# arnab39/equiadapt

Hardware: AMD Instinct MI355X
Metric: canonicalize+invert images/sec (224x224 C8) (higher is better)
Workload: dtype f32 (resampling / FFT / accumulation in fp32; the network's channel contraction as 2xfp16 split of every fp32 operand (within one fp32 ulp), 3 exact products, fp32 accumulate -- closer to fp64 than the fp32 matrix instruction, see step_ms_by_gemm_form); 1 GPU; configs[1]: 224x224x3 synthetic, C8, GroupEquivariantImageCanonicalization + ESCNNEquivariantNetwork in e2cnn's LAYER SHAPES (32 fields x 8 = 256 ch, k5, 3 layers, crop 0.8, resize 96) with this repository's own filter-bank parameterisation (bilinear-rotated banks; e2cnn's steerable basis is not restated -- e2cnn-trained weights enter via load_exported_dense), forward, then invert_canonicalization; batch_per_gpu=256, global_batch=256, parallelism=dp1 (no collective in the forward path)

## Files before the change

equiadapt_amd/csrc/lift_fft.hip:

```cpp
#include <cstdlib>

#include "eqa_common.hpp"

#ifndef EQA_LF_AUX
#define EQA_LF_AUX 2
#endif

namespace {

#include "fft_common.inc"

typedef float f32x4 __attribute__((ext_vector_type(4)));
typedef unsigned u32x4 __attribute__((ext_vector_type(4)));

struct alignas(4) LfPixel { float c[3]; };
__device__ __forceinline__ void lf_fetch_pixel(float (&p)[3], const float* __restrict__ x, unsigned off, bool ok) {
  const LfPixel v = *reinterpret_cast<const LfPixel*>(reinterpret_cast<const char*>(x) + (ok ? off : 0u));
#pragma unroll
  for (int c = 0; c < 3; ++c) p[c] = v.c[c];
}
__device__ __forceinline__ float lf_pixel_or_zero(float v, bool ok) { return ok ? v : 0.0f; }

#ifdef EQA_LF_CLOCK
__device__ unsigned long long g_lf_clock[64];
__device__ __forceinline__ int lf_clock_slot(int wave) { return wave == 8 ? 0 : wave == 1 ? 1 : wave == 0 ? 2 : wave == 6 ? 3 : wave == 11 ? 4 : -1; }
#define LF_CLOCK_BEGIN() const bool lfc_on = blockIdx.x == 0 && (threadIdx.x & 63) == 0 && lf_clock_slot(wave) >= 0; \
  if (blockIdx.x == 0 && (threadIdx.x & 63) == 0) { unsigned hw_; asm volatile("s_getreg_b32 %0, hwreg(HW_REG_HW_ID)" : "=s"(hw_)); g_lf_clock[40 + wave] = hw_; } \
  unsigned long long lfc_t = __builtin_readcyclecounter(); unsigned long long lfc_s[16] = {0, 0, 0, 0, 0, 0, 0, 0, 0, 0, 0, 0, 0, 0, 0, 0}
#define LF_CLOCK(i) do { const unsigned long long n_ = __builtin_readcyclecounter(); lfc_s[i] += n_ - lfc_t; lfc_t = n_; } while (0)
#define LF_CLOCK_END() do { if (lfc_on) for (int i_ = 0; i_ < 8; ++i_) g_lf_clock[8 * lf_clock_slot(wave) + i_] = lfc_s[i_]; } while (0)
#else
#define LF_CLOCK_BEGIN() do { } while (0)
#define LF_CLOCK(i) do { } while (0)
#define LF_CLOCK_END() do { } while (0)
#endif

constexpr int kLfThreads = 768;
constexpr int kLfCh = 16;
constexpr int kLfSteps = 19;
constexpr int kLfQuadPitch = 196;
constexpr int kLfRowPitch = 784;
constexpr int kLfTileFloats = kFftN * kLfRowPitch;
constexpr int kLfSubRows = 16;
constexpr int kLfPatchRows = kLfSubRows + 4, kLfPatchPitch = 156;
constexpr int kLfPatchFloats = kLfPatchRows * kLfPatchPitch;
constexpr int kLfLdsFloats = kLfTileFloats + kLfPatchFloats;
constexpr int kLfStagers = 6 * 64;
constexpr int kLfPre = (kLfPatchFloats + kLfStagers - 1) / kLfStagers;

__device__ __forceinline__ void lf_slot(int n, int& ky, int& e, bool& spare) {
  spare = n == 75;
  const bool lo = n < 70;
  const int r = n % 14;
  ky = lo ? n / 14 : min(n - 70, 4);
  e = lo ? (r >> 1) + 8 * (r & 1) : 7;
}

struct LfItem {
  unsigned grp, m;
  int gy0, gx0;
  size_t img;
};

__device__ __forceinline__ LfItem lf_item(unsigned work, int ngrp, int TY, int TX) {
  LfItem it;
  it.grp = work % ngrp;
#ifdef EQA_LF_XCDGRP
  if (ngrp == 16) it.grp = 2 * (it.grp % 8) + it.grp / 8;
#endif
  it.m = work / ngrp;
  const unsigned tx = it.m % TX, ty = (it.m / TX) % TY;
  it.img = it.m / ((unsigned)TX * TY);
  it.gy0 = kFftO * (int)ty;
  it.gx0 = kFftO * (int)tx;
  return it;
}

enum { kConv = 0, kCols = 1, kRowp = 2 };

#ifndef EQA_LF_H2_DEAL
#define EQA_LF_H2_DEAL 1
#endif
constexpr int kLhDeal = EQA_LF_H2_DEAL;
constexpr int kLhRun0 = kLhDeal == 0 ? 3 : 6, kLhRun1 = kLhDeal == 0 ? 6 : 0;
constexpr int kLhFirstConv = kLhDeal == 0 ? 8 : 6;
constexpr bool kLhConvRowsInTail = kLhDeal != 0;
struct LfRun { int y0, t0, y1, t1; bool cross; };
__host__ __device__ constexpr LfRun lf_h2_run(int wave, int ) {
  if (kLhDeal == 0) {
    const bool cross = wave == 9 || wave == 10;
    const int y0 = (wave == 8 || wave == 10) ? 0 : (wave == 9 ? 9 : 3), t0 = (wave == 8 || wave == 9) ? 0 : 2;
    return LfRun{y0, t0, cross ? (wave == 9 ? 0 : 6) : y0 + 3, cross ? 1 : t0, cross};
  }
  const bool lone = wave == 8 || wave == 9;
  const int y0 = ((lone ? wave == 9 : wave >= 10) ? 6 : 0), t0 = lone ? 0 : 1 + (wave & 1);
  return LfRun{y0, t0, y0 + kLhRun0, t0, false};
}
constexpr bool lf_h2_deal_covers() {
  int n[3][12] = {};
  for (int sub = 0; sub < 4; ++sub) {
    for (int w = kLhFirstConv; w < 12; ++w) {
      const LfRun r = lf_h2_run(w, sub);
      if (r.cross != (kLhRun1 > 0 && r.t1 != r.t0)) return false;
      for (int k = 0; k < kLhRun0 + kLhRun1; ++k) {
        const int y = k < kLhRun0 ? r.y0 + k : r.y1 + k - kLhRun0, t = k < kLhRun0 ? r.t0 : r.t1;
        if (y < 0 || y >= 12 || t < 0 || t >= 3) return false;
        ++n[t][y];
      }
    }
  }
  for (int t = 0; t < 3; ++t)
    for (int y = 0; y < 12; ++y)
      if (n[t][y] != 4) return false;
  return true;
}
static_assert(lf_h2_deal_covers(), "FORM 2: a tile of the sub-phase is left to no wave or taken by two");

#if EQA_LF_H2_DEAL != 0
__device__ __forceinline__ int lf_h2_rows(int wave, int s) { return s < 4 ? 0 : 4 * wave; }
#elif defined(EQA_LF_H2_ROWS_IN_SUB)
__device__ __forceinline__ int lf_h2_rows(int wave, int s) {
  if (s < 4) return wave == 6 ? (1 | ((s & 1) ? 4 : 0)) : (wave == 7 ? (2 | ((s & 1) ? 0 : 4)) : 0);
  return wave == 6 ? 36 : wave == 7 ? 40 : wave == 4 ? 44 : -1;
}
#else
__device__ __forceinline__ int lf_h2_rows(int wave, int s) {
  if (s < 4) return wave == 6 ? 1 : (wave == 7 ? 2 : 0);
  return wave == 6 ? 36 : wave == 7 ? 40 : wave == 0 ? 8 : wave == 4 ? 20 : wave == 1 ? 32 : wave == 5 ? 44 : -1;
}
#endif

template <class F, int... Is>
__device__ __forceinline__ void lf_for_const(F&& f, std::integer_sequence<int, Is...>) {
  (f(std::integral_constant<int, Is>()), ...);
}

constexpr int kLpRowB = 53 * 8;
constexpr int kLpPlaneB = 8 * kLpRowB;
constexpr int kLpPatchB = 3 * kLpPlaneB;
constexpr int kLpLdsBytes = kLfTileFloats * 4 + kLpPatchB;
constexpr int kLhRowB = 52 * 8;
constexpr int kLhRing = 16;
constexpr int kLhPlaneB = kLhRing * kLhRowB;
constexpr int kLhPatchB = 2 * kLhPlaneB;
constexpr int kLhLdsBytes = kLfTileFloats * 4 + kLhPatchB;
constexpr int kLhSubRows = 12;
constexpr int kLhPre = 3;
typedef _Float16 lf_f16x8 __attribute__((ext_vector_type(8)));
typedef _Float16 lf_f16x4 __attribute__((ext_vector_type(4)));
typedef __bf16 lf_bf16x8 __attribute__((ext_vector_type(8)));
typedef __bf16 lf_bf16x4 __attribute__((ext_vector_type(4)));
__device__ __forceinline__ void lf_split3(float x, __bf16& p1, __bf16& p2, __bf16& p3) {
  p1 = (__bf16)x;
  const float r1 = x - (float)p1;
  p2 = (__bf16)r1;
  p3 = (__bf16)(r1 - (float)p2);
}

template <int ROLE, int FORM>
__device__ __forceinline__ void lift5_fft48_body(const float* __restrict__ x, const float* __restrict__ bank, const float* __restrict__ bias,
                                                 int relu, float* __restrict__ V, int H0, int W0, int C, int TY, int TX, size_t Mp,
                                                 unsigned nwork, unsigned v_bytes, unsigned x_bytes, unsigned bank_bytes,
                                                 float* __restrict__ dcmax, const float* __restrict__ xbound, int nxbound, float w_scale) {
  constexpr bool COLS = ROLE == kCols;
  constexpr bool PIECES = FORM == 3;
  constexpr bool H2 = FORM == 2;
  constexpr int NSUB = PIECES ? 12 : (H2 ? 4 : 3);
  constexpr int SUBROWS = kFftN / NSUB;
  constexpr int NGRP = 12 / NSUB;
  extern __shared__ float lds[];
  float* const tile = lds;
  float* const patch = lds + kLfTileFloats;
  const int tid = threadIdx.x;
  const int lane = tid & 63;
  const int wave = __builtin_amdgcn_readfirstlane(tid >> 6);
  const int j = lane & 15, q = lane >> 4;
  const int ngrp = C / kLfCh;
  const int H1 = H0 - 4, W1 = W0 - 4;
  const unsigned nblk = gridDim.x;
  const unsigned patch_b = (unsigned)(kLfTileFloats * 4);
  LF_CLOCK_BEGIN();

  const __amdgpu_buffer_rsrc_t xr = __builtin_amdgcn_make_buffer_rsrc(const_cast<float*>(x), 0, x_bytes, 0x00020000);
  float pre[COLS ? kLfPre : 1];
  auto prefetch = [&](const LfItem& it, int sub, bool live) {
    if constexpr (COLS) {
      int tq = tid;
      asm volatile("" : "+v"(tq));
#pragma unroll
      for (int i = 0; i < kLfPre; ++i) {
        const int idx = tq + kLfStagers * i;
        const int pr = idx / kLfPatchPitch, pc = idx - pr * kLfPatchPitch;
        const int gy = it.gy0 + kLfSubRows * sub + pr, gxc = it.gx0 * 3 + pc;
        const bool ok = live && idx < kLfPatchFloats && gy < H0 && gxc < W0 * 3;
        const unsigned off = ok ? (unsigned)(((it.img * H0 + gy) * (size_t)(W0 * 3) + gxc) * 4) : 0xfffffff0u;
        pre[i] = __builtin_bit_cast(float, __builtin_amdgcn_raw_buffer_load_b32(xr, off, 0, 0));
      }
    }
  };
  auto stage = [&]() {
    if constexpr (COLS) {
#pragma unroll
      for (int i = 0; i < kLfPre; ++i) {
        const int idx = tid + kLfStagers * i;
        if (idx < kLfPatchFloats) patch[idx] = pre[i];
      }
    }
  };

  float preg[COLS && PIECES ? 2 : 1][3];
  bool preg_ok[2] = {false, false};
  auto prefetch_grp = [&](const LfItem& it, int g, int which, bool live) {
    if constexpr (COLS && PIECES) {
      int tq = tid;
      asm volatile("" : "+v"(tq));
      const int pr = tq / 52, px = tq - pr * 52;
      const int gy = it.gy0 + 4 * g + pr, gx = it.gx0 + px;
      preg_ok[which] = live && tq < 208 && gy < H0 && gx < W0;
      lf_fetch_pixel(preg[which], x, (unsigned)((((it.img * H0 + gy) * (size_t)W0 + gx) * 3) * 4), preg_ok[which]);
    }
  };
  auto stage_grp = [&](int g, int which) {
    if constexpr (COLS && PIECES) {
      if (tid < 208) {
        const int pr = tid / 52, px = tid - pr * 52;
        __bf16 pc[3][3];
#pragma unroll
        for (int c = 0; c < 3; ++c) lf_split3(lf_pixel_or_zero(preg[which][c], preg_ok[which]), pc[0][c], pc[1][c], pc[2][c]);
        char* dst = reinterpret_cast<char*>(lds) + patch_b + ((4 * g + pr) & 7) * kLpRowB + px * 8;
#pragma unroll
        for (int pl = 0; pl < 3; ++pl) {
          const lf_bf16x4 v = {pc[pl][0], pc[pl][1], pc[pl][2], (__bf16)0.0f};
          *reinterpret_cast<lf_bf16x4*>(dst + pl * kLpPlaneB) = v;
        }
      }
    }
  };

  float preh[(!COLS && H2) ? kLhPre : 1][3];
  unsigned preh_ok = 0;
  float x_scale = 1.0f, out_scale = 1.0f;
  if constexpr (H2) {
    float mx = 0.0f;
    for (int t = lane; t < nxbound; t += 64) mx = fmaxf(mx, xbound[t]);
#pragma unroll
    for (int o = 32; o > 0; o >>= 1) mx = fmaxf(mx, __shfl_xor(mx, o));
    int ex = 0;
    if (mx > 0.0f && mx < 3.0e38f) (void)frexpf(mx, &ex);
    ex = __builtin_amdgcn_readfirstlane(min(max(14 - ex, -100), 100));
    x_scale = ldexpf(1.0f, ex);
    out_scale = ldexpf(1.0f, -ex) / w_scale;
  }
  int h_pr[(!COLS && H2) ? kLhPre : 1], h_px[(!COLS && H2) ? kLhPre : 1];
  if constexpr (!COLS && H2) {
#pragma unroll
    for (int i = 0; i < kLhPre; ++i) {
      const int idx = tid - 6 * 64 + kLfStagers * i;
      h_pr[i] = idx / 52;
      h_px[i] = idx - h_pr[i] * 52;
    }
  }
  auto prefetch_h = [&](const LfItem& it, int row0, int nrows, bool live) {
    if constexpr (!COLS && H2) {
#ifdef EQA_LF_H2_NOPREFETCH
      if (row0 >= 0) return;
#endif
      preh_ok = 0;
#pragma unroll
      for (int i = 0; i < kLhPre; ++i) {
        const int pr = h_pr[i], px = h_px[i];
        const int gy = it.gy0 + row0 + pr, gx = it.gx0 + px;
        const bool ok = live && pr < nrows && gy < H0 && gx < W0;
        preh_ok |= ok ? 1u << i : 0u;
        lf_fetch_pixel(preh[i], x, (unsigned)((((it.img * H0 + gy) * (size_t)W0 + gx) * 3) * 4), ok);
      }
    }
  };
  auto stage_h = [&](int row0, int nrows) {
    if constexpr (!COLS && H2) {
#pragma unroll
      for (int i = 0; i < kLhPre; ++i) {
        asm volatile("" : "+v"(preh[i][0]), "+v"(preh[i][1]), "+v"(preh[i][2]));
        if (h_pr[i] < nrows) {
          const int pr = h_pr[i], px = h_px[i];
          _Float16 hi[3], lo[3];
#pragma unroll
          for (int c = 0; c < 3; ++c) {
            const float v = lf_pixel_or_zero(preh[i][c], (preh_ok >> i) & 1u) * x_scale;
            hi[c] = (_Float16)v;
            lo[c] = (_Float16)(v - (float)hi[c]);
          }
          char* dst = reinterpret_cast<char*>(lds) + patch_b + ((row0 + pr) & (kLhRing - 1)) * kLhRowB + px * 8;
          const lf_f16x4 vh = {hi[0], hi[1], hi[2], (_Float16)0.0f}, vl = {lo[0], lo[1], lo[2], (_Float16)0.0f};
          *reinterpret_cast<lf_f16x4*>(dst) = vh;
          *reinterpret_cast<lf_f16x4*>(dst + kLhPlaneB) = vl;
        }
      }
    }
  };

  const int nr = (wave == 10 || wave == 11) ? 2 : 3;
  const int r0 = wave == 8 ? 0 : (wave == 9 ? 3 : (wave == 6 ? 6 : (wave == 10 ? 9 : (wave == 7 ? 11 : 14))));
  unsigned a_off[kLfSteps];
  float wreg[kLfSteps];
  f32x4 bias4;
  auto setup = [&](const LfItem& it) {
    const __amdgpu_buffer_rsrc_t br = __builtin_amdgcn_make_buffer_rsrc(const_cast<float*>(bank), 0, bank_bytes, 0x00020000);
    const unsigned wb = (unsigned)((it.grp * kLfCh + j) * 75 * 4);
#pragma unroll
    for (int t = 0; t < kLfSteps; ++t) {
      int ky, e;
      bool spare;
      lf_slot(4 * t + q, ky, e, spare);
      a_off[t] = patch_b + (unsigned)(((r0 + ky) * kLfPatchPitch + j * 3 + e) * 4);
      wreg[t] = __builtin_bit_cast(float, __builtin_amdgcn_raw_buffer_load_b32(br, spare ? 0xfffffff0u : wb + (unsigned)((ky * 15 + e) * 4), 0, 0));
    }
#pragma unroll
    for (int r = 0; r < 4; ++r) bias4[r] = bias ? bias[it.grp * kLfCh + 4 * q + r] : 0.0f;
    asm volatile("" : "+v"(bias4));
  };
#ifndef EQA_LF_AHEAD
#define EQA_LF_AHEAD 5
#endif
  constexpr int kAhead = EQA_LF_AHEAD;
  auto conv_rows = [&](const LfItem& it, int y0) {
    float b[3][kLfSteps], bq[2][3][kAhead];
    auto lds_at = [&](int t, int drow, int tx3) {
#ifdef EQA_LF_NOLDSREAD
      return __builtin_bit_cast(float, a_off[t] + (unsigned)(drow + tx3));
#else
      return reinterpret_cast<const float*>(reinterpret_cast<const char*>(lds) + a_off[t])[drow * kLfPatchPitch + tx3 * 48];
#endif
    };
#pragma unroll
    for (int t = 0; t < kAhead; ++t)
#pragma unroll
      for (int tx3 = 0; tx3 < 3; ++tx3) bq[0][tx3][t] = lds_at(t, 0, tx3);
#pragma unroll
    for (int r = 0; r < 3; ++r) {
      if (r < nr) {
        const int par = r & 1;
        const bool row_ok = it.gy0 + y0 + r < H1;
        f32x4 acc[3] = {bias4, bias4, bias4};
        __builtin_amdgcn_sched_barrier(0);
#pragma unroll
        for (int t = 0; t < kLfSteps; ++t) {
#pragma unroll
          for (int tx3 = 0; tx3 < 3; ++tx3)
#ifdef EQA_LF_NOMFMA
            acc[tx3][t & 3] += wreg[t] * (t < kAhead ? bq[par][tx3][t] : b[tx3][t]);
#else
            acc[tx3] = __builtin_amdgcn_mfma_f32_16x16x4f32(wreg[t], t < kAhead ? bq[par][tx3][t] : b[tx3][t], acc[tx3], 0, 0, 0);
#endif
          __builtin_amdgcn_sched_barrier(0);
          if (t + kAhead < kLfSteps) {
#pragma unroll
            for (int tx3 = 0; tx3 < 3; ++tx3) b[tx3][t + kAhead] = lds_at(t + kAhead, r, tx3);
          } else if (r + 1 < nr) {
#pragma unroll
            for (int tx3 = 0; tx3 < 3; ++tx3) bq[par ^ 1][tx3][t + kAhead - kLfSteps] = lds_at(t + kAhead - kLfSteps, r + 1, tx3);
          }
          __builtin_amdgcn_sched_barrier(0);
        }
#pragma unroll
        for (int tx3 = 0; tx3 < 3; ++tx3) {
          const bool ok = row_ok && it.gx0 + tx3 * 16 + j < W1;
          f32x4 v = acc[tx3];
#pragma unroll
          for (int k = 0; k < 4; ++k) {
            float u = relu ? fmaxf(v[k], 0.0f) : v[k];
            v[k] = ok ? u : 0.0f;
          }
          *reinterpret_cast<f32x4*>(tile + (y0 + r) * kLfRowPitch + q * kLfQuadPitch + (tx3 * 16 + j) * 4) = v;
        }
      }
    }
  };

  lf_bf16x8 wq[PIECES ? 4 : 1][PIECES ? 3 : 1];
  unsigned c_off[PIECES ? 4 : 1];
  int c_ky[PIECES ? 4 : 1];
  auto setup_p = [&](const LfItem& it) {
    if constexpr (PIECES) {
      const __amdgpu_buffer_rsrc_t br = __builtin_amdgcn_make_buffer_rsrc(const_cast<float*>(bank), 0, bank_bytes, 0x00020000);
#pragma unroll
      for (int sstep = 0; sstep < 4; ++sstep) {
        const int c = 4 * sstep + q;
        c_ky[sstep] = min(c / 3, 4);
        c_off[sstep] = (unsigned)((j + 2 * (c % 3)) * 8);
#pragma unroll
        for (int wp = 0; wp < 3; ++wp) {
          const unsigned off = (unsigned)((((it.grp * kLfCh + j) * 3 + wp) * 16 + c) * 16);
          wq[sstep][wp] = __builtin_bit_cast(lf_bf16x8, __builtin_amdgcn_raw_buffer_load_b128(br, off, 0, 0));
        }
      }
#pragma unroll
      for (int r = 0; r < 4; ++r) bias4[r] = bias ? bias[it.grp * kLfCh + 4 * q + r] : 0.0f;
      asm volatile("" : "+v"(bias4));
    }
  };
  auto conv_tiles_p = [&](const LfItem& it, int y, int tx0, auto NT) {
    constexpr int nt = decltype(NT)::value;
    if constexpr (PIECES) {
      const bool row_ok = it.gy0 + y < H1;
      unsigned addr[4];
#pragma unroll
      for (int sstep = 0; sstep < 4; ++sstep) addr[sstep] = patch_b + (unsigned)(((y + c_ky[sstep]) & 7) * kLpRowB) + c_off[sstep] + (unsigned)(tx0 * 16 * 8);
      f32x4 acc[3] = {bias4, bias4, bias4};
      lf_bf16x8 bp[2][3][3];
      auto read_step = [&](int sstep, int buf) {
#pragma unroll
        for (int t = 0; t < 3; ++t)
          if (t < nt)
#pragma unroll
            for (int pl = 0; pl < 3; ++pl)
#ifdef EQA_LF_NOLDSREAD
            {
              const f32x4 cv = {1.0f + (float)(addr[sstep] & 7), 0.5f + t, 0.25f + pl, 2.0f};
              bp[buf][t][pl] = __builtin_bit_cast(lf_bf16x8, cv);
            }
#else
            {
              typedef unsigned long long u64x2_t __attribute__((ext_vector_type(2)));
              const unsigned long long* pp = reinterpret_cast<const unsigned long long*>(reinterpret_cast<const char*>(lds) + addr[sstep] + t * 128 + pl * kLpPlaneB);
              const u64x2_t two = {pp[0], pp[1]};
              bp[buf][t][pl] = __builtin_bit_cast(lf_bf16x8, two);
            }
#endif
      };
      read_step(0, 0);
#pragma unroll
      for (int sstep = 0; sstep < 4; ++sstep) {
        const int buf = sstep & 1;
        if (sstep + 1 < 4) read_step(sstep + 1, buf ^ 1);
        __builtin_amdgcn_sched_barrier(0);
        constexpr int kW[6] = {2, 0, 1, 1, 0, 0}, kP[6] = {0, 2, 1, 0, 1, 0};
#pragma unroll
        for (int pr = 0; pr < 6; ++pr) {
#pragma unroll
          for (int t = 0; t < 3; ++t)
            if (t < nt) acc[t] = __builtin_amdgcn_mfma_f32_16x16x32_bf16(wq[sstep][kW[pr]], bp[buf][t][kP[pr]], acc[t], 0, 0, 0);
          __builtin_amdgcn_sched_barrier(0);
        }
      }
#pragma unroll
      for (int t = 0; t < 3; ++t) {
        if (t < nt) {
          const int tx3 = tx0 + t;
          const bool ok = row_ok && it.gx0 + tx3 * 16 + j < W1;
          f32x4 v = acc[t];
#pragma unroll
          for (int k = 0; k < 4; ++k) {
            float u = relu ? fmaxf(v[k], 0.0f) : v[k];
            v[k] = ok ? u : 0.0f;
          }
          *reinterpret_cast<f32x4*>(tile + y * kLfRowPitch + q * kLfQuadPitch + (tx3 * 16 + j) * 4) = v;
        }
      }
    }
  };

  lf_f16x8 wh[H2 ? 5 : 1][H2 ? 2 : 1];
  int h_off = 0;
  auto setup_h = [&](const LfItem& it) {
    if constexpr (H2) {
      const __amdgpu_buffer_rsrc_t br = __builtin_amdgcn_make_buffer_rsrc(const_cast<float*>(bank), 0, bank_bytes, 0x00020000);
#pragma unroll
      for (int ky = 0; ky < 5; ++ky)
#pragma unroll
        for (int wp = 0; wp < 2; ++wp) {
          const unsigned off = (unsigned)(((((it.grp * kLfCh + j) * 2 + wp) * 5 + ky) * 4 + q) * 16);
          wh[ky][wp] = __builtin_bit_cast(lf_f16x8, __builtin_amdgcn_raw_buffer_load_b128(br, off, 0, 0));
        }
#pragma unroll
      for (int r = 0; r < 4; ++r) bias4[r] = bias ? bias[it.grp * kLfCh + 4 * q + r] : 0.0f;
      asm volatile("" : "+v"(bias4));
    }
  };
  auto conv_col_h = [&](const LfItem& it, auto N0, auto N1, int y0, int t0, int y1, int t1, bool cross_) {
    if constexpr (H2) {
      constexpr int NROWS = decltype(N0)::value + decltype(N1)::value, SW = decltype(N0)::value;
      static_assert(SW >= 2 && NROWS >= 2 && NROWS <= kLhSubRows, "a run: at least two rows, at most a tile column of the sub-phase");
      const bool cross = NROWS > SW && cross_;
#ifdef EQA_LF_H2_NOCONV
      return;
#endif
      const int base0 = (int)patch_b + (j - 1 + 2 * min(q, 2)) * 8 + t0 * 128;
      const int base1 = base0 + (t1 - t0) * 128;
      lf_f16x8 win[7][2];
      auto read_row = [&](int k, bool NEW) {
        const int a = (NEW ? base1 + ((y1 + k - SW) & (kLhRing - 1)) * kLhRowB : base0 + ((y0 + k) & (kLhRing - 1)) * kLhRowB);
#pragma unroll
        for (int pl = 0; pl < 2; ++pl) {
          typedef unsigned long long u64x2_t __attribute__((ext_vector_type(2)));
          const unsigned long long* pp = reinterpret_cast<const unsigned long long*>(reinterpret_cast<const char*>(lds) + a + pl * kLhPlaneB);
          const u64x2_t two = {pp[0], pp[1]};
          win[k % 7][pl] = __builtin_bit_cast(lf_f16x8, two);
        }
      };
#pragma unroll
      for (int k = 0; k < 6; ++k) read_row(k, false);
      const f32x4 zero = {0.0f, 0.0f, 0.0f, 0.0f};
      const bool col_ok0 = it.gx0 + t0 * 16 + j < W1, col_ok1 = it.gx0 + t1 * 16 + j < W1;
      f32x4 acc[2];
      f32x4 ev = zero;
      auto epi = [&](int m, int rp) {
        const int y = rp < SW ? y0 + rp : y1 + rp - SW;
        const int t = rp < SW ? t0 : t1;
        if (m == 0) ev = acc[rp & 1] * out_scale + bias4;
        else if (m == 1) { ev[0] = relu ? fmaxf(ev[0], 0.0f) : ev[0]; ev[1] = relu ? fmaxf(ev[1], 0.0f) : ev[1]; }
        else if (m == 2) { ev[2] = relu ? fmaxf(ev[2], 0.0f) : ev[2]; ev[3] = relu ? fmaxf(ev[3], 0.0f) : ev[3]; }
        else if (m == 3) {
          const bool ok = (rp < SW ? col_ok0 : col_ok1) && it.gy0 + y < H1;
#pragma unroll
          for (int k = 0; k < 4; ++k) ev[k] = ok ? ev[k] : 0.0f;
        } else if (m == 4) {
          *reinterpret_cast<f32x4*>(tile + y * kLfRowPitch + q * kLfQuadPitch + (t * 16 + j) * 4) = ev;
        }
      };
#pragma unroll
      for (int r = 0; r < NROWS; ++r) {
        if (r == SW && cross) {
          __builtin_amdgcn_sched_barrier(0);
#pragma unroll
          for (int k = SW; k < SW + 4; ++k) read_row(k, true);
        }
#pragma unroll
        for (int m = 0; m < 15; ++m) {
          const int ky = m / 3, ch = m % 3;
          __builtin_amdgcn_sched_barrier(0);
          acc[r & 1] = __builtin_amdgcn_mfma_f32_16x16x32_f16(wh[ky][ch == 0 ? 1 : 0], win[(r + ky) % 7][ch == 1 ? 1 : 0], m == 0 ? zero : acc[r & 1], 0, 0, 0);
          if (r > 0 && m >= 2 && m < 7) epi(m - 2, r - 1);
          if (m == 9 && r + 2 < NROWS) read_row(r + 6, r + 6 >= SW + 4);
        }
      }
      __builtin_amdgcn_sched_barrier(0);
#pragma unroll
      for (int m = 0; m < 5; ++m) epi(m, NROWS - 1);
    }
  };

  auto row_pass = [&](int y0) {
#ifdef EQA_LF_H2_NOROWP
    if (H2) return;
#endif
    float* const rowp = tile + (y0 + (lane >> 4)) * kLfRowPitch + ((lane & 15) >> 2) * kLfQuadPitch + (lane & 3);
    float re[kFftN], ore[kFftH], oim[kFftH];
#pragma unroll
    for (int xx = 0; xx < kFftN; ++xx) re[xx] = rowp[xx * 4];
    fft48_r2c(re, ore, oim);
#pragma unroll
    for (int k = 0; k < kFftH - 1; ++k) rowp[k * 4] = ore[k];
    rowp[24 * 4] = ore[24];
#pragma unroll
    for (int k = 1; k < kFftH - 1; ++k) rowp[(24 + k) * 4] = oim[k];
  };

  const int cw = COLS ? wave : 0;
  const int col_ci = lane >> 4, col_kxi = (lane >> 2) & 3, col_cq = lane & 3;
  const int kc_of0 = 8 * (cw >> 1) + 2 * (cw & 1) + (col_kxi >> 1);
  const int kc = kc_of0 + ((col_kxi & 1) ? 4 : 0);
  const bool odd = (col_kxi & 1) != 0;
  const bool has_packed = COLS && __builtin_amdgcn_readfirstlane((int)(cw == 0)) != 0;
  const bool pair_packed = COLS && kc_of0 == 0;
  const bool packed = COLS && kc == 0;
  const float* const colp = tile + col_cq * kLfQuadPitch + col_ci + kc * 4;
  const __amdgpu_buffer_rsrc_t vr = __builtin_amdgcn_make_buffer_rsrc(V, 0, v_bytes, 0x00020000);
  float cre[kFftN], cim[kFftN];
  unsigned pend_m = 0, pend_grp = 0;
  bool pending = false;
  float dc_seen = 0.0f;
  auto transpose4 = [&](float& r0_, float& r1_, float& r2_, float& r3_) {
    auto sw16 = [](float& a, float& b) { asm volatile("s_nop 1\n\tv_permlane16_swap_b32 %0, %1" : "+v"(a), "+v"(b)); };
    auto sw32 = [](float& a, float& b) { asm volatile("s_nop 1\n\tv_permlane32_swap_b32 %0, %1" : "+v"(a), "+v"(b)); };
    sw16(r0_, r1_);
    sw16(r2_, r3_);
    sw32(r0_, r2_);
    sw32(r1_, r3_);
  };
  auto swz4 = [](float v) { return __builtin_bit_cast(float, __builtin_amdgcn_ds_swizzle(__builtin_bit_cast(int, v), 0x101f)); };
  auto store_pair = [&](float* re, float* im, unsigned voff1, unsigned voff2, bool second) {
    transpose4(re[0], re[1], re[2], re[3]);
    transpose4(im[0], im[1], im[2], im[3]);
    f32x4 o1, o2;
#pragma unroll
    for (int r = 0; r < 4; ++r) {
      const float got = swz4(odd ? re[r] : im[r]);
      o1[r] = odd ? got : re[r];
      o2[r] = odd ? im[r] : got;
    }
    __builtin_amdgcn_raw_buffer_store_b128(__builtin_bit_cast(u32x4, o1), vr, voff1, 0, EQA_LF_AUX);
    if (second) __builtin_amdgcn_raw_buffer_store_b128(__builtin_bit_cast(u32x4, o2), vr, voff2, 0, EQA_LF_AUX);
  };
  auto col_work = [&](auto SUB) {
    constexpr int sub = decltype(SUB)::value;
    if (!pending) return;
#ifdef EQA_LF_H2_NOCOLS
    if (H2) return;
#endif
    const size_t rowb = Mp * 2 * (size_t)C * 4;
    const unsigned col = (unsigned)(((size_t)pend_m * 2 * C + pend_grp * 2 * kLfCh) * 4) + (unsigned)((odd ? 64 : 0) + 16 * col_cq);
    if (sub == 0) {
      float ore[kFftN], oim[kFftN];
      fft48(cre, cim, ore, oim);
#pragma unroll
      for (int ky = 0; ky < kFftN; ++ky) {
        cre[ky] = ore[ky];
        cim[ky] = oim[ky];
      }
      if (has_packed) {
        float p24re[28], p24im[28];
#pragma unroll
        for (int ky = 0; ky < kFftH; ++ky) {
          const int kn = (kFftN - ky) % kFftN;
          const float a = ore[ky], b = oim[ky], c2 = ore[kn], d = oim[kn];
          p24re[ky] = 0.5f * (b + d);
          p24im[ky] = 0.5f * (c2 - a);
          cre[ky] = packed ? 0.5f * (a + c2) : a;
          cim[ky] = packed ? 0.5f * (b - d) : b;
        }
        dc_seen = fmaxf(dc_seen, packed ? cre[0] : 0.0f);
#pragma unroll
        for (int ky = kFftH; ky < 28; ++ky) p24re[ky] = p24im[ky] = 0.0f;
#ifndef EQA_LF_NOSTORE
        const unsigned vb24 = (unsigned)((size_t)(kFftN * kFftInner + 1 + 2 * col_ci) * rowb) + col;
#pragma unroll
        for (int g = 0; g < 7; ++g) {
          const bool live = pair_packed && 4 * g + col_ci < kFftH;
          store_pair(&p24re[4 * g], &p24im[4 * g], live ? vb24 + (unsigned)g * (unsigned)(8 * rowb) : 0xfffffff0u, 0xfffffff0u, false);
        }
#endif
      }
    }
#ifndef EQA_LF_NOSTORE
    const unsigned f1 = pair_packed ? (unsigned)(kFftN * kFftInner + 2 * col_ci) : (unsigned)(kFftInner * col_ci + kc_of0 - 1);
    const unsigned vb1 = (unsigned)((size_t)f1 * rowb) + col, vs1 = (unsigned)((pair_packed ? 8 : 4 * kFftInner) * rowb);
    const unsigned vb2 = (unsigned)((size_t)(kFftInner * col_ci + kc_of0 + 3) * rowb) + col, vs2 = (unsigned)(4 * kFftInner * rowb);
#pragma unroll
    for (int g = NGRP * sub; g < NGRP * sub + NGRP; ++g) {
      const bool live1 = !pair_packed || 4 * g + col_ci < kFftH;
      store_pair(&cre[4 * g], &cim[4 * g], live1 ? vb1 + (unsigned)g * vs1 : 0xfffffff0u, vb2 + (unsigned)g * vs2, true);
    }
#endif
  };

  unsigned cur_grp = 0xffffffffu;
  unsigned v = blockIdx.x;
  if constexpr (PIECES) {
    if (COLS && tid < 24) *reinterpret_cast<unsigned long long*>(reinterpret_cast<char*>(lds) + patch_b + tid * kLpRowB + 52 * 8) = 0ull;
    const LfItem f = lf_item(v < nwork ? v : 0, ngrp, TY, TX);
    prefetch_grp(f, 0, 0, v < nwork);
    prefetch_grp(f, 1, 1, v < nwork);
    stage_grp(0, 0);
    stage_grp(1, 1);
  } else if constexpr (H2) {
    if (tid == 0) *reinterpret_cast<unsigned long long*>(reinterpret_cast<char*>(lds) + patch_b - 8) = 0ull;
    prefetch_h(lf_item(v < nwork ? v : 0, ngrp, TY, TX), 0, kLhRing, v < nwork);
    stage_h(0, kLhRing);
    __syncthreads();
  } else {
    if (v < nwork) prefetch(lf_item(v, ngrp, TY, TX), 0, true);
    stage();
    __syncthreads();
  }
  for (;; v += nblk) {
    const bool live = v < nwork;
    if (!live && !pending) break;
    const LfItem it = lf_item(live ? v : 0, ngrp, TY, TX);
    const unsigned vn = v + nblk;
    const bool next_live = live && vn < nwork;
    const LfItem nx = lf_item(next_live ? vn : 0, ngrp, TY, TX);
    if constexpr (!COLS) {
#pragma unroll 1
      for (int sub = 0; sub < NSUB; ++sub) {
        if (PIECES || sub > 0) __syncthreads();
        LF_CLOCK(0);
        if constexpr (H2) {
          if (sub < NSUB - 1) prefetch_h(it, kLhSubRows * sub + kLhRing, kLhSubRows, live);
          else prefetch_h(nx, 0, kLhRing, next_live);
          LF_CLOCK(1);
        }
        if (live) {
          if (sub == 0 && it.grp != cur_grp) {
            if constexpr (PIECES) setup_p(it);
            else if constexpr (H2) { if constexpr (ROLE == kConv) setup_h(it); }
            else setup(it);
            cur_grp = it.grp;
          }
          if constexpr (H2) {
            if constexpr (ROLE == kConv) {
              const int y = kLhSubRows * sub;
              const LfRun run = lf_h2_run(wave, sub);
              conv_col_h(it, std::integral_constant<int, kLhRun0>(), std::integral_constant<int, kLhRun1>(), y + run.y0, run.t0, y + run.y1, run.t1,
                         run.cross);
            } else {
              if (sub > 0) {
                const int a = lf_h2_rows(wave, sub);
#pragma unroll 1
                for (int k = 0; k < 3; ++k)
                  if (a & (1 << k)) row_pass(kLhSubRows * (sub - 1) + 4 * k);
              }
            }
          } else if constexpr (PIECES) {
            const int y = SUBROWS * sub + (wave == 8 ? 0 : (wave == 9 ? 1 : ((wave == 6 || wave == 10) ? 2 : 3)));
            const int tx0 = (wave == 10 || wave == 11) ? 2 : 0;
            if (wave == 8 || wave == 9) conv_tiles_p(it, y, tx0, std::integral_constant<int, 3>());
            else if (wave == 10 || wave == 11) conv_tiles_p(it, y, tx0, std::integral_constant<int, 1>());
            else conv_tiles_p(it, y, tx0, std::integral_constant<int, 2>());
          } else {
            conv_rows(it, kLfSubRows * sub + r0);
            if (sub > 0 && (wave == 8 || wave == 9)) row_pass(8 * (sub - 1) + 4 * (wave - 8));
          }
        }
        LF_CLOCK(2);
        __syncthreads();
        LF_CLOCK(3);
        if constexpr (H2) {
          if (sub < NSUB - 1) stage_h(kLhSubRows * sub + kLhRing, kLhSubRows);
          else stage_h(0, kLhRing);
        }
      }
    } else {
      auto subphase = [&](auto SUB) {
        constexpr int sub = decltype(SUB)::value;
        if constexpr (FORM == 0) {
          if (sub > 0) stage();
        }
        if (PIECES || sub > 0) __syncthreads();
        LF_CLOCK(0);
        if constexpr (H2) {
        } else if constexpr (PIECES) {
          if (sub < NSUB - 1) {
            prefetch_grp(it, sub + 2, 0, live);
          } else {
            prefetch_grp(nx, 0, 0, next_live);
            prefetch_grp(nx, 1, 1, next_live);
          }
        } else {
          if (sub < NSUB - 1) prefetch(it, sub + 1, live);
          else prefetch(nx, 0, next_live);
        }
        LF_CLOCK(1);
        col_work(SUB);
        LF_CLOCK(2);
        __syncthreads();
        LF_CLOCK(3);
        if constexpr (PIECES) {
          if (sub < NSUB - 1) {
            stage_grp(sub + 2, 0);
          } else {
            stage_grp(0, 0);
            stage_grp(1, 1);
          }
        }
      };
      lf_for_const(subphase, std::make_integer_sequence<int, NSUB>());
      if constexpr (FORM == 0) stage();
    }
    if constexpr (PIECES) {
      if (live) row_pass(4 * wave);
    } else if constexpr (H2) {
      if constexpr (ROLE != kConv || kLhConvRowsInTail) {
        const int a = lf_h2_rows(wave, NSUB);
        if (live && a >= 0) row_pass(a);
      }
    } else {
      if (live && wave < 8) row_pass(16 + 4 * wave);
    }
    LF_CLOCK(4);
    __syncthreads();
    LF_CLOCK(5);
    constexpr int kEarly = PIECES ? kFftN : (H2 ? kLhSubRows : kLfSubRows);
    if constexpr (COLS) {
      if (live) {
#pragma unroll
        for (int y = 0; y < kEarly; ++y) {
          cre[y] = colp[y * kLfRowPitch];
          cim[y] = colp[y * kLfRowPitch + 24 * 4];
        }
      }
    }
    LF_CLOCK(6);
    __syncthreads();
    LF_CLOCK(7);
    if constexpr (COLS && !PIECES) {
      if (live) {
#pragma unroll
        for (int y = kEarly; y < kFftN; ++y) {
          cre[y] = colp[y * kLfRowPitch];
          cim[y] = colp[y * kLfRowPitch + 24 * 4];
        }
      }
    }
    pend_m = it.m;
    pend_grp = it.grp;
    pending = live;
  }
  if constexpr (COLS) {
    if (dcmax != nullptr && has_packed) {
      float m = dc_seen;
#pragma unroll
      for (int o = 32; o > 0; o >>= 1) m = fmaxf(m, __shfl_xor(m, o));
      if (lane == 0) dcmax[blockIdx.x] = m;
      if (blockIdx.x == 0) {
        for (unsigned t = nblk + lane; t < (unsigned)EQA_LIFT5_DCMAX_SLOTS; t += 64) dcmax[t] = 0.0f;
      }
    }
  }
  LF_CLOCK_END();
}

__global__ __launch_bounds__(kLfThreads) void lift5_fft48_fused_kernel(const float* __restrict__ x, const float* __restrict__ bank,
                                                                        const float* __restrict__ bias, int relu, float* __restrict__ V,
                                                                        int H0, int W0, int C, int TY, int TX, size_t Mp, unsigned nwork,
                                                                        unsigned v_bytes, unsigned x_bytes, unsigned bank_bytes,
                                                                        float* __restrict__ dcmax) {
  if (threadIdx.x < 6 * 64) lift5_fft48_body<kCols, 0>(x, bank, bias, relu, V, H0, W0, C, TY, TX, Mp, nwork, v_bytes, x_bytes, bank_bytes, dcmax, nullptr, 0, 1.0f);
  else lift5_fft48_body<kConv, 0>(x, bank, bias, relu, V, H0, W0, C, TY, TX, Mp, nwork, v_bytes, x_bytes, bank_bytes, dcmax, nullptr, 0, 1.0f);
}

__global__ __launch_bounds__(kLfThreads) void lift5_fft48_fused_pieces_kernel(const float* __restrict__ x, const float* __restrict__ bank,
                                                                               const float* __restrict__ bias, int relu, float* __restrict__ V,
                                                                               int H0, int W0, int C, int TY, int TX, size_t Mp, unsigned nwork,
                                                                               unsigned v_bytes, unsigned x_bytes, unsigned bank_bytes,
                                                                               float* __restrict__ dcmax) {
  if (threadIdx.x < 6 * 64) lift5_fft48_body<kCols, 3>(x, bank, bias, relu, V, H0, W0, C, TY, TX, Mp, nwork, v_bytes, x_bytes, bank_bytes, dcmax, nullptr, 0, 1.0f);
  else lift5_fft48_body<kConv, 3>(x, bank, bias, relu, V, H0, W0, C, TY, TX, Mp, nwork, v_bytes, x_bytes, bank_bytes, dcmax, nullptr, 0, 1.0f);
}

__global__ __launch_bounds__(kLfThreads) void lift5_fft48_fused_h2_kernel(const float* __restrict__ x, const float* __restrict__ bank,
                                                                           const float* __restrict__ bias, int relu, float* __restrict__ V,
                                                                           int H0, int W0, int C, int TY, int TX, size_t Mp, unsigned nwork,
                                                                           unsigned v_bytes, unsigned x_bytes, unsigned bank_bytes,
                                                                           float* __restrict__ dcmax, const float* __restrict__ xbound,
                                                                           int nxbound, float w_scale) {
  const int w = __builtin_amdgcn_readfirstlane((int)(threadIdx.x >> 6));
  if (w < 6) lift5_fft48_body<kCols, 2>(x, bank, bias, relu, V, H0, W0, C, TY, TX, Mp, nwork, v_bytes, x_bytes, bank_bytes, dcmax, xbound, nxbound, w_scale);
  else if (w >= kLhFirstConv) lift5_fft48_body<kConv, 2>(x, bank, bias, relu, V, H0, W0, C, TY, TX, Mp, nwork, v_bytes, x_bytes, bank_bytes, dcmax, xbound, nxbound, w_scale);
  else if constexpr (kLhFirstConv > 6) lift5_fft48_body<kRowp, 2>(x, bank, bias, relu, V, H0, W0, C, TY, TX, Mp, nwork, v_bytes, x_bytes, bank_bytes, dcmax, xbound, nxbound, w_scale);
#ifdef EQA_LF_CLOCK
  if (blockIdx.x == 0 && threadIdx.x == 0) g_lf_clock[63] = 1 + kLhDeal;
#endif
}

__global__ __launch_bounds__(256) void absmax_slots_kernel(const float* __restrict__ x, size_t n, float* __restrict__ out) {
  float m = 0.0f;
  const size_t n4 = n / 4;
  for (size_t i = (size_t)blockIdx.x * 256 + threadIdx.x; i < n4; i += (size_t)gridDim.x * 256) {
    const f32x4 v = reinterpret_cast<const f32x4*>(x)[i];
    m = fmaxf(fmaxf(m, fmaxf(fabsf(v[0]), fabsf(v[1]))), fmaxf(fabsf(v[2]), fabsf(v[3])));
  }
  if (blockIdx.x == 0 && threadIdx.x < (n & 3)) m = fmaxf(m, fabsf(x[n4 * 4 + threadIdx.x]));
  __shared__ float red[4];
#pragma unroll
  for (int o = 32; o > 0; o >>= 1) m = fmaxf(m, __shfl_xor(m, o));
  if ((threadIdx.x & 63) == 0) red[threadIdx.x >> 6] = m;
  __syncthreads();
  if (threadIdx.x == 0) out[blockIdx.x] = fmaxf(fmaxf(red[0], red[1]), fmaxf(red[2], red[3]));
}

}

extern "C" {

#ifdef EQA_LF_CLOCK
int eqa_debug_lf_clock(unsigned long long* out) { return hipMemcpyFromSymbol(out, HIP_SYMBOL(g_lf_clock), sizeof(g_lf_clock)) == hipSuccess ? 0 : -1; }
#endif

int eqa_lift5_fft48k5_input_supported(int Cin, int KH, int KW, int Cout) {
  return (Cin == 3 && KH == 5 && KW == 5 && Cout > 0 && Cout % kLfCh == 0) ? 1 : 0;
}

static int lift_fft_launch(const float* x, const void* bank, size_t bank_bytes, const float* bias, int relu, float* V, int nimg, int H0, int W0,
                           int Cout, void* stream, bool pieces, float* dcmax = nullptr, const float* xbound = nullptr, int nxbound = 0,
                           float w_scale = 0.0f) {
  if (!x || !bank || !V || nimg < 0 || H0 < 5 || W0 < 5 || Cout <= 0) return EQA_ERR_INVALID_ARG;
  if (Cout % kLfCh != 0) return EQA_ERR_UNSUPPORTED;
  if (nimg == 0) return EQA_OK;
  const int H1 = H0 - 4, W1 = W0 - 4;
  const int TY = (int)eqa_fft48k5_tiles(H1), TX = (int)eqa_fft48k5_tiles(W1);
  if (TY <= 0 || TX <= 0) return EQA_ERR_UNSUPPORTED;
  const size_t M = (size_t)nimg * TY * TX;
  const size_t nwork = M * (Cout / kLfCh);
  const size_t vb = (size_t)kFftF * fft_pitch(M) * 2 * Cout * 4;
  const size_t xb = (size_t)nimg * H0 * W0 * 3 * 4;
  if (nwork > 0x7fffffffULL || vb > 0xffffff00ULL || xb > 0xffffff00ULL || bank_bytes > 0xffffff00ULL) return EQA_ERR_UNSUPPORTED;
  const bool h2 = xbound != nullptr;
  const void* kern = h2 ? (const void*)lift5_fft48_fused_h2_kernel : pieces ? (const void*)lift5_fft48_fused_pieces_kernel : (const void*)lift5_fft48_fused_kernel;
  const int lds_bytes = h2 ? kLhLdsBytes : pieces ? kLpLdsBytes : kLfLdsFloats * 4;
  if (!allow_dynamic_lds(kern, lds_bytes)) return EQA_ERR_UNSUPPORTED;
  const unsigned ngrp = (unsigned)(Cout / kLfCh);
  unsigned nblk = 256;
  if (ngrp <= 256) nblk = (256 / ngrp) * ngrp;
  if ((size_t)nblk > nwork) nblk = (unsigned)nwork;
  if (h2)
    hipLaunchKernelGGL(lift5_fft48_fused_h2_kernel, dim3(nblk), dim3(kLfThreads), lds_bytes, (hipStream_t)stream, x, (const float*)bank, bias,
                       relu, V, H0, W0, Cout, TY, TX, fft_pitch(M), (unsigned)nwork, (unsigned)vb, (unsigned)xb, (unsigned)bank_bytes, dcmax,
                       xbound, nxbound, w_scale);
  else if (pieces)
    hipLaunchKernelGGL(lift5_fft48_fused_pieces_kernel, dim3(nblk), dim3(kLfThreads), lds_bytes, (hipStream_t)stream, x, (const float*)bank, bias,
                       relu, V, H0, W0, Cout, TY, TX, fft_pitch(M), (unsigned)nwork, (unsigned)vb, (unsigned)xb, (unsigned)bank_bytes, dcmax);
  else
    hipLaunchKernelGGL(lift5_fft48_fused_kernel, dim3(nblk), dim3(kLfThreads), lds_bytes, (hipStream_t)stream, x, (const float*)bank, bias,
                       relu, V, H0, W0, Cout, TY, TX, fft_pitch(M), (unsigned)nwork, (unsigned)vb, (unsigned)xb, (unsigned)bank_bytes, dcmax);
  return launch_status();
}

int eqa_lift5_fft48k5_input(const float* x, const float* bank, const float* bias, int relu, float* V, int nimg, int H0, int W0, int Cout,
                            void* stream) {
  return lift_fft_launch(x, bank, (size_t)(Cout > 0 ? Cout : 0) * 75 * 4, bias, relu, V, nimg, H0, W0, Cout, stream, false);
}

int eqa_lift5_fft48k5_input_dcmax(const float* x, const float* bank, const float* bias, int relu, float* V, float* dcmax, int nimg, int H0,
                                  int W0, int Cout, void* stream) {
  if (!dcmax) return EQA_ERR_INVALID_ARG;
  if (!relu) return EQA_ERR_UNSUPPORTED;
  if (nimg == 0) return hipMemsetAsync(dcmax, 0, EQA_LIFT5_DCMAX_SLOTS * sizeof(float), (hipStream_t)stream) == hipSuccess ? EQA_OK : EQA_ERR_LAUNCH;
  return lift_fft_launch(x, bank, (size_t)(Cout > 0 ? Cout : 0) * 75 * 4, bias, relu, V, nimg, H0, W0, Cout, stream, false, dcmax);
}

int64_t eqa_lift5_pieces_f16_bytes(int Cout) { return Cout > 0 ? (int64_t)Cout * 2 * 5 * 4 * 8 * 2 : 0; }

int eqa_absmax_slots(const float* x, int64_t n, float* slots, void* stream) {
  if (n < 0 || !slots || (n > 0 && !x)) return EQA_ERR_INVALID_ARG;
  if (((uintptr_t)x & 15) != 0) return EQA_ERR_UNSUPPORTED;
  hipLaunchKernelGGL(absmax_slots_kernel, dim3(EQA_LIFT5_DCMAX_SLOTS), dim3(256), 0, (hipStream_t)stream, x, (size_t)n, slots);
  return launch_status();
}

int eqa_lift5_fft48k5_input_f16x2(const float* x, const void* wpieces, float w_scale, const float* xbound, int nxbound, const float* bias,
                                  int relu, float* V, float* dcmax, int nimg, int H0, int W0, int Cout, void* stream) {
  if (!xbound || nxbound <= 0 || !(w_scale > 0.0f)) return EQA_ERR_INVALID_ARG;
  int ex = 0;
  if (frexpf(w_scale, &ex) != 0.5f) return EQA_ERR_INVALID_ARG;
  if (dcmax && !relu) return EQA_ERR_UNSUPPORTED;
  if (nimg == 0 && dcmax) return hipMemsetAsync(dcmax, 0, EQA_LIFT5_DCMAX_SLOTS * sizeof(float), (hipStream_t)stream) == hipSuccess ? EQA_OK : EQA_ERR_LAUNCH;
  return lift_fft_launch(x, wpieces, (size_t)eqa_lift5_pieces_f16_bytes(Cout), bias, relu, V, nimg, H0, W0, Cout, stream, false, dcmax, xbound,
                         nxbound, w_scale);
}

int64_t eqa_lift5_pieces_bytes(int Cout) { return Cout > 0 ? (int64_t)Cout * 3 * 16 * 8 * 2 : 0; }

int eqa_lift5_fft48k5_input_bf16x3(const float* x, const void* wpieces, const float* bias, int relu, float* V, int nimg, int H0, int W0,
                                   int Cout, void* stream) {
  return lift_fft_launch(x, wpieces, (size_t)eqa_lift5_pieces_bytes(Cout), bias, relu, V, nimg, H0, W0, Cout, stream, true);
}

}
```

Measured before the change: 74350 images/s.

## Move half of FORM-2 row passes into sub-phase windows on column waves

Under the default H2 deal, row passes were previously all run in the tail after the last sub-phase, one per wave across all 12 waves. The new default row deal (3) gives six of the twelve row passes to waves 1 and 4 inside sub-phases 1-3, as soon as their rows have been convolved. The other six go to the column waves 0-5 in the tail, and the conv waves 6-11 no longer run any. The aim is to overlap row-pass work with the sub-phase windows and shorten the serialized tail before the final barrier. The cost is that waves 1 and 4 get longer inside those windows, which may stretch the barriers. A compile-time check verifies that every row pass is run exactly once and only after its rows are ready. The clock probe instrumentation is widened at the same time.

```diff
diff --git a/equiadapt_amd/csrc/lift_fft.hip b/equiadapt_amd/csrc/lift_fft.hip
--- a/equiadapt_amd/csrc/lift_fft.hip
+++ b/equiadapt_amd/csrc/lift_fft.hip
@@ -22,13 +22,14 @@
 __device__ __forceinline__ float lf_pixel_or_zero(float v, bool ok) { return ok ? v : 0.0f; }
 
 #ifdef EQA_LF_CLOCK
-__device__ unsigned long long g_lf_clock[64];
-__device__ __forceinline__ int lf_clock_slot(int wave) { return wave == 8 ? 0 : wave == 1 ? 1 : wave == 0 ? 2 : wave == 6 ? 3 : wave == 11 ? 4 : -1; }
+__device__ unsigned long long g_lf_clock[128];
+__device__ __forceinline__ int lf_clock_slot(int wave) { return wave == 8 ? 0 : wave == 1 ? 1 : wave == 0 ? 2 : wave == 6 ? 3 : wave == 11 ? 4 : wave == 2 ? 5 : -1; }
 #define LF_CLOCK_BEGIN() const bool lfc_on = blockIdx.x == 0 && (threadIdx.x & 63) == 0 && lf_clock_slot(wave) >= 0; \
   if (blockIdx.x == 0 && (threadIdx.x & 63) == 0) { unsigned hw_; asm volatile("s_getreg_b32 %0, hwreg(HW_REG_HW_ID)" : "=s"(hw_)); g_lf_clock[40 + wave] = hw_; } \
-  unsigned long long lfc_t = __builtin_readcyclecounter(); unsigned long long lfc_s[16] = {0, 0, 0, 0, 0, 0, 0, 0, 0, 0, 0, 0, 0, 0, 0, 0}
-#define LF_CLOCK(i) do { const unsigned long long n_ = __builtin_readcyclecounter(); lfc_s[i] += n_ - lfc_t; lfc_t = n_; } while (0)
-#define LF_CLOCK_END() do { if (lfc_on) for (int i_ = 0; i_ < 8; ++i_) g_lf_clock[8 * lf_clock_slot(wave) + i_] = lfc_s[i_]; } while (0)
+  unsigned long long lfc_t = __builtin_readcyclecounter(); unsigned lfc_s[9] = {0, 0, 0, 0, 0, 0, 0, 0, 0}
+#define LF_CLOCK(i) do { const unsigned long long n_ = __builtin_readcyclecounter(); lfc_s[i] += (unsigned)(n_ - lfc_t); lfc_t = n_; } while (0)
+#define LF_CLOCK_END() do { if (lfc_on) { const int k_ = lf_clock_slot(wave); \
+  for (int i_ = 0; i_ < 8; ++i_) g_lf_clock[(k_ < 5 ? 8 * k_ : 64) + i_] = lfc_s[i_]; g_lf_clock[72 + k_] = lfc_s[8]; } } while (0)
 #else
 #define LF_CLOCK_BEGIN() do { } while (0)
 #define LF_CLOCK(i) do { } while (0)
@@ -84,7 +85,6 @@
 constexpr int kLhDeal = EQA_LF_H2_DEAL;
 constexpr int kLhRun0 = kLhDeal == 0 ? 3 : 6, kLhRun1 = kLhDeal == 0 ? 6 : 0;
 constexpr int kLhFirstConv = kLhDeal == 0 ? 8 : 6;
-constexpr bool kLhConvRowsInTail = kLhDeal != 0;
 struct LfRun { int y0, t0, y1, t1; bool cross; };
 __host__ __device__ constexpr LfRun lf_h2_run(int wave, int ) {
   if (kLhDeal == 0) {
@@ -117,7 +117,50 @@
 static_assert(lf_h2_deal_covers(), "FORM 2: a tile of the sub-phase is left to no wave or taken by two");
 
 #if EQA_LF_H2_DEAL != 0
-__device__ __forceinline__ int lf_h2_rows(int wave, int s) { return s < 4 ? 0 : 4 * wave; }
+#ifndef EQA_LF_H2_ROWDEAL
+#define EQA_LF_H2_ROWDEAL 3
+#endif
+constexpr int kLhRowDeal = EQA_LF_H2_ROWDEAL;
+static_assert(kLhRowDeal == 0 || kLhRowDeal == 3, "EQA_LF_H2_ROWDEAL: 0 or 3 (1 and 2 were measured and removed: profiles/r17)");
+__host__ __device__ constexpr int lf_h2_rowmask(int wave, int s) {
+  if (kLhRowDeal == 0) return s < 4 ? 0 : 1 << wave;
+  if (s < 4) return s < 1 ? 0 : wave == 1 ? 1 << (2 * (s - 1)) : wave == 4 ? 1 << (2 * (s - 1) + 1) : 0;
+  return wave < 6 ? 1 << (6 + wave) : 0;
+}
+constexpr bool lf_h2_rowdeal_covers() {
+  int n[12] = {};
+  for (int s = 0; s <= 4; ++s)
+    for (int w = 0; w < 12; ++w) {
+      const int m = lf_h2_rowmask(w, s);
+      if (m & ~0xfff) return false;
+      if (s < 4 && w >= 6 && m) return false;
+      if (m & (m - 1)) return false;
+      for (int k = 0; k < 12; ++k)
+        if (m & (1 << k)) {
+          if (s <= k / 3) return false;
+          ++n[k];
+        }
+    }
+  for (int k = 0; k < 12; ++k)
+    if (n[k] != 1) return false;
+  return true;
+}
+static_assert(lf_h2_rowdeal_covers(), "FORM 2: a row pass is run by no wave or by two, or in a window in which its rows are not convolved yet");
+constexpr bool lf_h2_window_has_pass(int s) {
+  for (int w = 0; w < 6; ++w)
+    if (lf_h2_rowmask(w, s)) return true;
+  return false;
+}
+constexpr bool lf_h2_conv_rows_in_tail() {
+  for (int w = 6; w < 12; ++w)
+    if (lf_h2_rowmask(w, 4)) return true;
+  return false;
+}
+__device__ __forceinline__ int lf_h2_rows(int wave, int s) {
+  if (kLhRowDeal == 0 && s == 4) return 4 * wave;
+  const int m = lf_h2_rowmask(wave, s);
+  return m ? 4 * __builtin_ctz(m) : -1;
+}
 #elif defined(EQA_LF_H2_ROWS_IN_SUB)
 __device__ __forceinline__ int lf_h2_rows(int wave, int s) {
   if (s < 4) return wave == 6 ? (1 | ((s & 1) ? 4 : 0)) : (wave == 7 ? (2 | ((s & 1) ? 0 : 4)) : 0);
@@ -128,6 +171,10 @@
   if (s < 4) return wave == 6 ? 1 : (wave == 7 ? 2 : 0);
   return wave == 6 ? 36 : wave == 7 ? 40 : wave == 0 ? 8 : wave == 4 ? 20 : wave == 1 ? 32 : wave == 5 ? 44 : -1;
 }
+#endif
+#if EQA_LF_H2_DEAL == 0
+constexpr bool lf_h2_window_has_pass(int) { return false; }
+constexpr bool lf_h2_conv_rows_in_tail() { return false; }
 #endif
 
 template <class F, int... Is>
@@ -743,6 +790,13 @@
         LF_CLOCK(1);
         col_work(SUB);
         LF_CLOCK(2);
+        if constexpr (H2) {
+          if constexpr (sub > 0 && lf_h2_window_has_pass(sub)) {
+            const int a = lf_h2_rows(wave, sub);
+            if (live && a >= 0) row_pass(a);
+            LF_CLOCK(8);
+          }
+        }
         __syncthreads();
         LF_CLOCK(3);
         if constexpr (PIECES) {
@@ -760,7 +814,7 @@
     if constexpr (PIECES) {
       if (live) row_pass(4 * wave);
     } else if constexpr (H2) {
-      if constexpr (ROLE != kConv || kLhConvRowsInTail) {
+      if constexpr (ROLE != kConv || lf_h2_conv_rows_in_tail()) {
         const int a = lf_h2_rows(wave, NSUB);
         if (live && a >= 0) row_pass(a);
       }
@@ -839,7 +893,12 @@
   else if (w >= kLhFirstConv) lift5_fft48_body<kConv, 2>(x, bank, bias, relu, V, H0, W0, C, TY, TX, Mp, nwork, v_bytes, x_bytes, bank_bytes, dcmax, xbound, nxbound, w_scale);
   else if constexpr (kLhFirstConv > 6) lift5_fft48_body<kRowp, 2>(x, bank, bias, relu, V, H0, W0, C, TY, TX, Mp, nwork, v_bytes, x_bytes, bank_bytes, dcmax, xbound, nxbound, w_scale);
 #ifdef EQA_LF_CLOCK
-  if (blockIdx.x == 0 && threadIdx.x == 0) g_lf_clock[63] = 1 + kLhDeal;
+  if (blockIdx.x == 0 && threadIdx.x == 0) {
+    g_lf_clock[63] = 1 + kLhDeal;
+#if EQA_LF_H2_DEAL != 0
+    g_lf_clock[62] = 1 + kLhRowDeal;
+#endif
+  }
 #endif
 }
 
```

After: 75530 images/s (median of 6 runs). +1.6%, better.
